# arbellea/LSTM-UNet

Measured on AMD Instinct MI355X. Metric: training frames/sec (seq_len*batch) at 256x256, higher is better.
Workload: dtype f32

## Files before the change

lstm-unet_amd/csrc/lu_conv.hip:

```cpp
#include <stdarg.h>
#include <stdlib.h>
#include <string.h>
#include <stdio.h>
#include <type_traits>
#include <utility>
#include "lu_device.h"

namespace {

constexpr int CK = 16;
constexpr int BM = 256;
constexpr int A_LD = CK + 4;

struct SrcInfo {
    const float* x;
    const float* w;
    int64_t frame_stride;
    int64_t w_tap_stride;
    int32_t pix_stride, C, w_row_stride;
    int32_t thin;
    int32_t nchunk;
    int32_t bf16;
};

// ... 234 lines not shown
            rok = row < CK && j < a.kk * si.C;
            tap = j / si.C;
            c = j - tap * si.C;
        }
        const float* wp = si.w + (int64_t)tap * si.w_tap_stride + (int64_t)c * si.w_row_stride + bcol;
        if (BVEC) {
            const bool ok = rok && ((EPI == LU_EPI_LSTM) || bcol < a.N);
            return *reinterpret_cast<const float4*>(ok ? wp : zp);
        } else {
            const float t0 = *((rok && bcol + 0 < a.N) ? wp + 0 : zp), t1 = *((rok && bcol + 1 < a.N) ? wp + 1 : zp),
                        t2 = *((rok && bcol + 2 < a.N) ? wp + 2 : zp), t3 = *((rok && bcol + 3 < a.N) ? wp + 3 : zp);
            return make_float4(t0, t1, t2, t3);
        }
    };
    auto load_weights = [&](const SrcInfo& si, bool thin, int tap_v, int chunk) {
        rb0 = load_w(si, thin, tap_v, chunk, 0);
        if (NPB > 1) rb1 = load_w(si, thin, tap_v, chunk, 1);
    };
    int64_t rowoff[RA];
#pragma unroll
    for (int i = 0; i < RA; ++i) rowoff[i] = 0;
    int cached_s = -1;
    auto load_stage = [&](const IterState& st) {
        const SrcInfo& si = a.src[st.s];
        const int c = st.chunk * CK + 4 * q;
        const bool cok = c < si.C;
        const float* pv[RA];
        if (GEN) {
#pragma unroll
            for (int i = 0; i < RA; ++i) {
                const int vy = vy0[i] + st.kh, vx = vx0[i] + st.kw;
                const int iy = vy >> a.dsh, ix = vx >> a.dsh;
                const bool ok = cok && vy >= 0 && vx >= 0 && iy < a.Hin && ix < a.Win && ((vy | vx) & a.dsh) == 0;
                const float* p = si.x + (int64_t)fr[i] * si.frame_stride + ((int64_t)iy * a.Win + ix) * si.pix_stride + c;
                pv[i] = ok ? p : zp;
            }
        } else {
            if (st.s != cached_s) {
                cached_s = st.s;
#pragma unroll
                for (int i = 0; i < RA; ++i)
                    rowoff[i] = (int64_t)fr[i] * si.frame_stride + ((int64_t)vy0[i] * a.Win + vx0[i]) * si.pix_stride;
            }
            const float* tapbase = si.x + ((int64_t)st.kh * a.Win + st.kw) * si.pix_stride + c;
#pragma unroll
            for (int i = 0; i < RA; ++i) {
                const bool ok = cok && (unsigned)(vy0[i] + st.kh) < (unsigned)a.Hin &&
                                (unsigned)(vx0[i] + st.kw) < (unsigned)a.Win;
                pv[i] = ok ? tapbase + rowoff[i] : zp;
            }
        }
#pragma unroll
        for (int i = 0; i < RA; ++i) ra[i] = *reinterpret_cast<const float4*>(pv[i]);
        load_weights(si, false, st.tap, st.chunk);
    };
    auto dma_stage = [&](const IterState& st, int buf) {
        const SrcInfo& si = a.src[st.s];
        if (!GEN && st.s != cached_s) {
            cached_s = st.s;
#pragma unroll
            for (int i = 0; i < RA; ++i)
                rowoff[i] = (int64_t)fr[i] * si.frame_stride + ((int64_t)vy0[i] * a.Win + vx0[i]) * si.pix_stride;
        }
        const float* tapbase = si.x + ((int64_t)st.kh * a.Win + st.kw) * si.pix_stride;
#pragma unroll
        for (int i = 0; i < RA; ++i) {
            const int row = (tid >> 2) + (NT / 4) * i;
            const int c = st.chunk * CK + 4 * (q ^ ((row >> 2) & 3));
            const float* p;
            bool ok;
            if (GEN) {
                const int vy = vy0[i] + st.kh, vx = vx0[i] + st.kw;
                const int iy = vy >> a.dsh, ix = vx >> a.dsh;
                ok = c < si.C && vy >= 0 && vx >= 0 && iy < a.Hin && ix < a.Win && ((vy | vx) & a.dsh) == 0;
                p = si.x + (int64_t)fr[i] * si.frame_stride + ((int64_t)iy * a.Win + ix) * si.pix_stride + c;
            } else {
                ok = c < si.C && (unsigned)(vy0[i] + st.kh) < (unsigned)a.Hin && (unsigned)(vx0[i] + st.kw) < (unsigned)a.Win;
                p = tapbase + rowoff[i] + c;
            }
            lu_glds16(ok ? p : zp, &As[buf][(wave * 16 + (NT / 4) * i) * ALD]);
        }
#pragma unroll
        for (int pp = 0; pp < NPB; ++pp) {
            const int row = brow0 + RPP * pp;
            const int c = st.chunk * CK + row;
            const bool ok = row < CK && c < si.C && ((EPI == LU_EPI_LSTM) || bcol < a.N);
            const float* wp = si.w + (int64_t)st.tap * si.w_tap_stride + (int64_t)c * si.w_row_stride + bcol;
            if (RPP * (pp + 1) <= CK || row < CK) lu_glds16(ok ? wp : zp, &Bs[buf][(wave * 64 + NT * pp) * 4]);
        }
    };

    auto load_thin = [&](const SrcInfo& si, int chunk) {
        const int kkC = a.kk * si.C;
        int dy[4], dx[4], cc[4];
        bool jok[4];
#pragma unroll
        for (int e = 0; e < 4; ++e) {
            int j = chunk * CK + 4 * q + e;
            jok[e] = j < kkC;
            int tap = j / si.C;
            cc[e] = j - tap * si.C;
            dy[e] = tap / a.k;
            dx[e] = tap - dy[e] * a.k;
        }
#pragma unroll
        for (int i = 0; i < RA; ++i) {
            float v[4];
#pragma unroll
            for (int e = 0; e < 4; ++e) {
                const int vy = vy0[i] + dy[e], vx = vx0[i] + dx[e];
                const int iy = vy >> a.dsh, ix = vx >> a.dsh;
                const bool ok = jok[e] && vy >= 0 && vx >= 0 && iy < a.Hin && ix < a.Win && ((vy | vx) & a.dsh) == 0;
                const float* p = si.x + (int64_t)fr[i] * si.frame_stride + ((int64_t)iy * a.Win + ix) * si.pix_stride + cc[e];
                v[e] = *(ok ? p : zp);
            }
            ra[i] = make_float4(v[0], v[1], v[2], v[3]);
        }
        load_weights(si, true, 0, chunk);
    };

    auto store_stage = [&](int buf) {
#pragma unroll
        for (int i = 0; i < RA; ++i)
        {
            const int row = (tid >> 2) + (NT / 4) * i;
            const int slot = DMA ? (q ^ ((row >> 2) & 3)) : q;
            *reinterpret_cast<float4*>(&As[buf][row * ALD + 4 * slot]) = ra[i];
        }
        if (RPP <= CK || brow0 < CK) *reinterpret_cast<float4*>(&Bs[buf][brow0 * BN + 4 * bq]) = rb0;
        if (NPB > 1) *reinterpret_cast<float4*>(&Bs[buf][(brow0 + RPP) * BN + 4 * bq]) = rb1;
    };

    f32x16 acc[MF][NF];
#pragma unroll
    for (int mf = 0; mf < MF; ++mf)
#pragma unroll
        for (int nf = 0; nf < NF; ++nf)
#pragma unroll
            for (int r = 0; r < 16; ++r) acc[mf][nf][r] = 0.f;

    const int arow = wave * (32 * MF) + (lane & 31);
    const int khalf = 4 * (lane >> 5);
    float4 afr[MF][2];
    float bvr[2][NF];
    auto rd_af = [&](int buf, int s) {
#pragma unroll
        for (int mf = 0; mf < MF; ++mf) {
            const int row = arow + 32 * mf;
            const int grp = 2 * s + (khalf >> 2);
            const int slot = DMA ? (grp ^ ((row >> 2) & 3)) : grp;
            afr[mf][s] = *reinterpret_cast<const float4*>(&As[buf][row * ALD + 4 * slot]);
        }
    };
    auto rd_bv = [&](int buf, int g) {
        const int s = g >> 2, j = g & 3;
#pragma unroll
        for (int nf = 0; nf < NF; ++nf) bvr[g & 1][nf] = Bs[buf][(8 * s + khalf + j) * BN + 32 * nf + (lane & 31)];
    };
    auto stage_begin = [&](int buf) {
        rd_af(buf, 0);
        rd_bv(buf, 0);
        rd_af(buf, 1);
    };
    auto mma_group = [&](int buf, int g) {
        const int s = g >> 2, j = g & 3;
        if (g + 1 < 8) rd_bv(buf, g + 1);
#pragma unroll
        for (int mf = 0; mf < MF; ++mf) {
            const float4& fa = afr[mf][s];
            const float av = j == 0 ? fa.x : j == 1 ? fa.y : j == 2 ? fa.z : fa.w;
#pragma unroll
            for (int nf = 0; nf < NF; ++nf) acc[mf][nf] = lu_mfma(av, bvr[g & 1][nf], acc[mf][nf]);
        }
    };
    auto mma_stage = [&](int buf) {
        stage_begin(buf);
#pragma unroll
        for (int g = 0; g < 8; ++g) mma_group(buf, g);
    };

    for (int ts = 0; ts < (ks == 0 ? a.n_thin : 0); ++ts) {
        const SrcInfo& si = a.tsrc[ts];
        for (int ch = 0; ch < si.nchunk; ++ch) {
            load_thin(si, ch);
            store_stage(0);
            __syncthreads();
            mma_stage(0);
            __syncthreads();
        }
    }

    int it0 = 0, it1 = a.n_it;
    if (a.ksplit > 1) {
        const int per = (a.n_it + a.ksplit - 1) / a.ksplit;
        it0 = ks * per;
        it1 = it0 + per < a.n_it ? it0 + per : a.n_it;
    }
    if (it1 > it0) {
        IterState st{0, 0, 0, 0, 0};
        {
            int r = it0;
            while (r >= a.src[st.s].nchunk * a.kk) {
                r -= a.src[st.s].nchunk * a.kk;
                ++st.s;
            }
            st.chunk = r / a.kk;
            st.tap = r - st.chunk * a.kk;
            st.kh = st.tap / a.k;
            st.kw = st.tap - st.kh * a.k;
        }
        if (DMA) {
            dma_stage(st, 0);
        } else {
            load_stage(st);
            store_stage(0);
        }
        __syncthreads();
        for (int it = it0; it < it1; ++it) {
            const int buf = (it - it0) & 1;
            stage_begin(buf);
            mma_group(buf, 0);
            LU_SCHED_FENCE();
            if (it + 1 < it1) iter_advance(st, a);
            if (DMA) {
                if (!LU_DBG(a, 1)) dma_stage(st, buf ^ 1);
                LU_SCHED_FENCE();
#pragma unroll
                for (int g = 1; g < 8; ++g) {
                    mma_group(buf, g);
                    LU_SCHED_FENCE();
                }
            } else {
                if (!LU_DBG(a, 1)) load_stage(st);
                LU_SCHED_FENCE();
#pragma unroll
                for (int g = 1; g < 7; ++g) {
                    mma_group(buf, g);
                    LU_SCHED_FENCE();
                }
                if (!LU_DBG(a, 2)) store_stage(buf ^ 1);
                LU_SCHED_FENCE();
                mma_group(buf, 7);
            }
            if (!LU_DBG(a, 4)) __syncthreads();
        }
    }

    if (EPI == LU_EPI_BIAS && a.out_vec4s && a.ksplit <= 1) {
        float* const Exw = &As[0][0] + wave * (16 * 36);
        const int cq = lane & 7;
#pragma unroll
        for (int mf = 0; mf < MF; ++mf)
#pragma unroll
            for (int half = 0; half < 2; ++half) {
                int64_t obase[2];
                bool rok[2];
#pragma unroll
                for (int q = 0; q < 2; ++q) {
                    const int64_t m = m0 + wave * (32 * MF) + mf * 32 + 16 * half + (lane >> 3) + 8 * q;
                    rok[q] = m < a.M;
                    RowCursor rc;
                    rc.set(a, rok[q] ? m : 0);
                    obase[q] = (int64_t)rc.f * a.out_frame_stride +
                               (a.out_row_stride ? (int64_t)rc.oy * a.out_row_stride + (int64_t)rc.ox * a.out_pix_stride
                                                 : (int64_t)rc.pix * a.out_pix_stride);
                }
#pragma unroll
                for (int nf = 0; nf < NF; ++nf) {
#pragma unroll
                    for (int rr = 0; rr < 8; ++rr)
                        Exw[((rr & 3) + 8 * (rr >> 2) + 4 * (lane >> 5)) * 36 + (lane & 31)] = acc[mf][nf][8 * half + rr];
                    LU_WAVE_SYNC();
                    const int col = n0 + 32 * nf + 4 * cq;
                    const float4 bq = (a.bias && col < a.N) ? *reinterpret_cast<const float4*>(a.bias + col) : make_float4(0.f, 0.f, 0.f, 0.f);
#pragma unroll
                    for (int q = 0; q < 2; ++q) {
                        float4 v = *reinterpret_cast<const float4*>(&Exw[((lane >> 3) + 8 * q) * 36 + 4 * cq]);
                        v.x += bq.x; v.y += bq.y; v.z += bq.z; v.w += bq.w;
                        if (rok[q] && col < a.N) *reinterpret_cast<float4*>(a.out + obase[q] + col) = v;
                    }
                    LU_WAVE_SYNC();
                }
            }
        return;
    }
#pragma unroll
    for (int mf = 0; mf < MF; ++mf) {
        const int64_t mb = m0 + wave * (32 * MF) + mf * 32 + 4 * (lane >> 5);
        RowCursor rc;
        rc.set(a, mb < a.M ? mb : 0);
#pragma unroll
        for (int r = 0; r < 16; ++r) {
            if (r) rc.advance(a, (r & 3) ? 1 : 5);
            const int64_t m = mb + (r & 3) + 8 * (r >> 2);
            if (m >= a.M) continue;
            float v[NF];
#pragma unroll
            for (int nf = 0; nf < NF; ++nf) v[nf] = acc[mf][nf][r];
            conv_epilogue_row<NF, EPI>(a, v, rc.f, rc.pix, m, nt, n0, ks, lane & 31, rc.oy);
        }
    }
}

template <int K, int EPI, bool ST = false>
__global__ __launch_bounds__(512, 4) void conv_halo_kernel(ConvArgs a) {
    const float* const lu_z16 = a.zero16 ? a.zero16 : lu_zero16;
    constexpr int NF = 4, BN = 128, NT = 512, TH = 8, TW = 32;
    constexpr int HWD = TW + K - 1, HHT = TH + K - 1, HP = HHT * HWD;
    constexpr int HPASS = (HP * 4 + NT - 1) / NT;
    constexpr int PAD = (K - 1) / 2;
    static_assert(HP * A_LD >= BM * A_LD, "halo buffer doubles as the [256][20] tile of the thin-source prologue");
    __shared__ __attribute__((aligned(16))) float Ah[HP * A_LD];
    __shared__ __attribute__((aligned(16))) float Bs[3][CK * BN];

    const int tid = threadIdx.x, lane = tid & 63, wave = tid >> 6;
    const int bid = blockIdx.x;
    const int slot = bid >> 3;
    int tile, nt, ks;
    const bool live = lu_block_tile(a, tile, nt, ks);
    if (a.xcd_by_n) {
        const int g = a.n_tiles >> 3;
        nt = (bid & 7) * g + (slot % g);
        tile = slot / g;
        if (tile >= a.m_tiles) return;
    } else if (!live) {
        return;
    }
    const int f = tile / a.tiles_pf;
    const int t2 = tile - f * a.tiles_pf;
    const int y0 = (t2 / a.tiles_x) * TH, x0 = (t2 % a.tiles_x) * TW;
    const int n0 = nt * BN;
    const float* const zp = lu_z16;
    const float* const x_s0 = a.src[0].x + (int64_t)f * a.src[0].frame_stride;
    const float* const x_s1 = a.src[1].x + (int64_t)f * a.src[1].frame_stride;
    const float* const w_s0 = a.src[0].w;
    const float* const w_s1 = a.src[1].w;
    const int64_t wts_s0 = a.src[0].w_tap_stride, wts_s1 = a.src[1].w_tap_stride;
    const int wrs_s0 = a.src[0].w_row_stride, wrs_s1 = a.src[1].w_row_stride;
    const int ps_s0 = a.src[0].pix_stride, ps_s1 = a.src[1].pix_stride;
    const int C_s0 = a.src[0].C, C_s1 = a.src[1].C;
    const int nch_s0 = a.src[0].nchunk, nch_s1 = a.src[1].nchunk;
    const int q = tid & 3;
    const int bq = tid & 31, brow = tid >> 5;
    const int bcol = (EPI == LU_EPI_LSTM) ? (bq >> 3) * a.F + nt * 32 + 4 * (bq & 7) : n0 + 4 * bq;

    lu_u4 rh[HPASS];
    float4 rb = make_float4(0.f, 0.f, 0.f, 0.f);
    auto load_halo = [&](int src, int chunk) {
        const int c = chunk * CK + 4 * q;
        const float* base = (src ? x_s1 : x_s0) + c;
        const int ps = src ? ps_s1 : ps_s0;
        const bool cok = c < (src ? C_s1 : C_s0);
#pragma unroll
        for (int i = 0; i < HPASS; ++i) {
            const int hp = (tid + NT * i) >> 2;
            const int hy = hp / HWD, hx = hp - hy * HWD;
            const int iy = y0 + hy - PAD, ix = x0 + hx - PAD;
            const bool ok = cok && hp < HP && iy >= 0 && iy < a.Hin && ix >= 0 && ix < a.Win;
            const float* p = base + (int64_t)(iy * a.Win + ix) * ps;
            rh[i] = *reinterpret_cast<const lu_u4*>(ok ? p : zp);
        }
    };
    auto store_halo = [&]() {
#pragma unroll
        for (int i = 0; i < HPASS; ++i) {
            const int hp = (tid + NT * i) >> 2;
            if (hp < HP) *reinterpret_cast<lu_u4*>(&Ah[hp * A_LD + 4 * q]) = rh[i];
        }
    };
    auto load_b = [&](const SrcInfo& si, bool thin, int tap_v, int chunk) {
        int tap, c;
        bool rok;
        if (!thin) {
            tap = tap_v;
            c = chunk * CK + brow;
            rok = c < si.C;
        } else {
            const int j = chunk * CK + brow;
            rok = j < a.kk * si.C;
            tap = j / si.C;
            c = j - tap * si.C;
        }
        const float* wp = si.w + (int64_t)tap * si.w_tap_stride + (int64_t)c * si.w_row_stride + bcol;
        const bool ok = rok && ((EPI == LU_EPI_LSTM) || bcol < a.N);
        rb = *reinterpret_cast<const float4*>(ok ? wp : zp);
    };
    int d_s = 0, d_chunk = 0, d_tap = 0;
    int64_t d_wts = 0;
    const float* wq = nullptr;
    bool wok = false;
    const bool colok = (EPI == LU_EPI_LSTM) || bcol < a.N;
    auto dma_seek = [&](int src, int chunk, int tap) {
        d_s = src;
        d_chunk = chunk;
        d_tap = tap;
        const int c = chunk * CK + brow;
        wq = (src ? w_s1 : w_s0) + (int64_t)tap * (src ? wts_s1 : wts_s0) + (int64_t)c * (src ? wrs_s1 : wrs_s0) + bcol;
        wok = c < (src ? C_s1 : C_s0) && colok;
        d_wts = src ? wts_s1 : wts_s0;
    };
    auto dma_next = [&](float* Bd) {
        lu_glds16(wok ? wq : zp, Bd + wave * 256);
        if (++d_tap < K * K) {
            wq += d_s ? wts_s1 : wts_s0;
        } else if (d_chunk + 1 < (d_s ? nch_s1 : nch_s0)) {
            dma_seek(d_s, d_chunk + 1, 0);
        } else {
            dma_seek(d_s + 1, 0, 0);
        }
    };
    auto dma_issue = [&](float* Bd, int mode) {
        if (mode == 0) {
            dma_next(Bd);
            return;
        }
        lu_glds16(wok ? wq : zp, Bd + wave * 256);
        if (mode == 1) wq += d_wts;
        else if (d_chunk + 1 < (d_s ? nch_s1 : nch_s0)) dma_seek(d_s, d_chunk + 1, 0);
        else dma_seek(d_s + 1, 0, 0);
    };
    auto store_b = [&](int buf) { *reinterpret_cast<float4*>(&Bs[buf][brow * BN + 4 * bq]) = rb; };

    f32x16 acc[NF];
#pragma unroll
    for (int nf = 0; nf < NF; ++nf)
#pragma unroll
        for (int r = 0; r < 16; ++r) acc[nf][r] = 0.f;

    const int khalf = 4 * (lane >> 5);
    const int boff = khalf * BN + (lane & 31);
    struct B4 {
        float x, y, z, w;
    };
    auto rd_b = [&](const float* Br, int g) {
        if (EPI == LU_EPI_BIAS) {
            const float4 v = *reinterpret_cast<const float4*>(Br + khalf * BN + 4 * (lane & 31) + (8 * (g >> 2) + (g & 3)) * BN);
            return B4{v.x, v.y, v.z, v.w};
        }
        const float* p = Br + boff + (8 * (g >> 2) + (g & 3)) * BN;
        return B4{p[0], p[32], p[64], p[96]};
    };
    auto rd_a = [&](int arow, int s) { return *reinterpret_cast<const float4*>(&Ah[arow * A_LD + 8 * s + khalf]); };
    auto mma4 = [&](float av, const B4& b) {
        acc[0] = lu_mfma(av, b.x, acc[0]);
        acc[1] = lu_mfma(av, b.y, acc[1]);
        acc[2] = lu_mfma(av, b.z, acc[2]);
        acc[3] = lu_mfma(av, b.w, acc[3]);
    };
    float4 fa0, fa1;
    B4 fb[2];
    auto fa_of = [&](int g) {
        const float4& fa = (g >> 2) ? fa1 : fa0;
        const int j = g & 3;
        return j == 0 ? fa.x : j == 1 ? fa.y : j == 2 ? fa.z : fa.w;
    };
    auto simple_stage = [&](const float* Br, int arow) {
        fa0 = rd_a(arow, 0);
        fa1 = rd_a(arow, 1);
#pragma unroll
        for (int g = 0; g < 8; ++g) {
            fb[0] = rd_b(Br, g);
            mma4(fa_of(g), fb[0]);
        }
    };

    if (ks == 0) {
        const int oyr[2] = {y0 + ((tid >> 2) >> 5), y0 + (((tid >> 2) + 128) >> 5)};
        const int oxr = x0 + ((tid >> 2) & 31);
        for (int ts = 0; ts < a.n_thin; ++ts) {
            const SrcInfo& si = a.tsrc[ts];
            const int kkC = a.kk * si.C;
            for (int ch = 0; ch < si.nchunk; ++ch) {
                float4 rt[2];
#pragma unroll
                for (int i = 0; i < 2; ++i) {
                    float v[4];
#pragma unroll
                    for (int e = 0; e < 4; ++e) {
                        const int jj = ch * CK + 4 * q + e;
                        const int tap = jj / si.C, cc = jj - tap * si.C;
                        const int dy = tap / K, dx = tap - dy * K;
                        const int iy = oyr[i] + dy - PAD, ix = oxr + dx - PAD;
                        const bool ok = jj < kkC && oyr[i] < a.Hin && oxr < a.Win && iy >= 0 && iy < a.Hin && ix >= 0 &&
                                        ix < a.Win;
                        const float* p = si.x + (int64_t)f * si.frame_stride + ((int64_t)iy * a.Win + ix) * si.pix_stride + cc;
                        v[e] = *(ok ? p : zp);
                    }
                    rt[i] = make_float4(v[0], v[1], v[2], v[3]);
                }
                load_b(si, true, 0, ch);
#pragma unroll
                for (int i = 0; i < 2; ++i)
                    *reinterpret_cast<float4*>(&Ah[((tid >> 2) + 128 * i) * A_LD + 4 * q]) = rt[i];
                store_b(0);
                __syncthreads();
                simple_stage(&Bs[0][0], wave * 32 + (lane & 31));
                __syncthreads();
            }
        }
    }

    int it0 = 0, it1 = a.n_it;
    if (a.ksplit > 1) {
        const int per = ST ? ((a.n_it / (K * K) + a.ksplit - 1) / a.ksplit) * (K * K) : (a.n_it + a.ksplit - 1) / a.ksplit;
        it0 = ks * per < a.n_it ? ks * per : a.n_it;
        it1 = it0 + per < a.n_it ? it0 + per : a.n_it;
    }
    if (it1 > it0) {
        IterState st{0, 0, 0, 0, 0};
        {
            int r = it0;
            while (r >= a.src[st.s].nchunk * a.kk) {
                r -= a.src[st.s].nchunk * a.kk;
                ++st.s;
            }
            st.chunk = r / a.kk;
            st.tap = r - st.chunk * a.kk;
            st.kh = st.tap / K;
            st.kw = st.tap - st.kh * K;
        }
        int c_s = st.s, c_chunk = st.chunk, tap = st.tap, kw = st.kw, aoff = st.kh * HWD + st.kw;
        auto next_chunk = [&](int& ns, int& nc) {
            ns = c_s;
            nc = c_chunk + 1;
            if (nc == (c_s ? nch_s1 : nch_s0)) {
                nc = 0;
                ++ns;
            }
        };
        load_halo(c_s, c_chunk);
        dma_seek(c_s, c_chunk, tap);
        dma_next(&Bs[0][0]);
        if (it0 + 1 < it1) dma_next(&Bs[1][0]);
        store_halo();
        if (it0 + 1 < it1 && tap == K * K - 1) {
            int ns, nc;
            next_chunk(ns, nc);
            load_halo(ns, nc);
        }
        __syncthreads();
        auto stage_sync = [&](int vm, bool lds) {
#ifdef LU_EMU
            __syncthreads();
#else
            if (lds) {
                if (vm == 0) __builtin_amdgcn_s_waitcnt(0x0070);
                else __builtin_amdgcn_s_waitcnt(0x0071);
            } else {
                if (vm == 0) __builtin_amdgcn_s_waitcnt(0x0F70);
                else __builtin_amdgcn_s_waitcnt(0x0F70 | HPASS);
            }
            __builtin_amdgcn_s_barrier();
#endif
        };
        auto stage = [&](float* __restrict__ Bd, const float* __restrict__ Br, const float* __restrict__ Bn, int arow, int arow_n,
                         bool dma, int dmode, bool halo_ld, bool halo_st, bool more) {
            fb[1] = rd_b(Br, 1);
            fa1 = rd_a(arow, 1);
            mma4(fa0.x, fb[0]);
            LU_SCHED_FENCE();
            if (halo_ld) {
                int ns, nc;
                next_chunk(ns, nc);
                load_halo(ns, nc);
            }
            LU_SCHED_FENCE();
#pragma unroll
            for (int g = 1; g < 4; ++g) {
                fb[(g + 1) & 1] = rd_b(Br, g + 1);
                mma4(fa_of(g), fb[g & 1]);
                LU_SCHED_FENCE();
            }
            if (!halo_st) {
                stage_sync(halo_ld ? 1 : 0, false);
                if (dma) dma_issue(Bd, dmode);
            }
            LU_SCHED_FENCE();
#pragma unroll
            for (int g = 4; g < 8; ++g) {
                if (g < 7) fb[(g + 1) & 1] = rd_b(Br, g + 1);
                else if (more && !halo_st) fb[0] = rd_b(Bn, 0);
                if (g == 5 && more && !halo_st) fa0 = rd_a(arow_n, 0);
                mma4(fa_of(g), fb[g & 1]);
                LU_SCHED_FENCE();
            }
            if (halo_st) {
#ifdef LU_EMU
                __syncthreads();
#else
                __builtin_amdgcn_s_barrier();
#endif
                store_halo();
                if (dma) dma_issue(Bd, dmode);
                stage_sync(dma ? 1 : 0, true);
                if (more) {
                    fa0 = rd_a(arow_n, 0);
                    fb[0] = rd_b(Bn, 0);
                }
            }
        };
        int b0 = 0, b1 = 1, b2 = 2;
        const int arow0 = wave * HWD + (lane & 31);
        fa0 = rd_a(arow0 + aoff, 0);
        fb[0] = rd_b(&Bs[0][0], 0);
        if constexpr (ST) {
            const int n_chunks = (it1 - it0) / (K * K);
            auto rotate = [&]() {
                const int t = b0;
                b0 = b1;
                b1 = b2;
                b2 = t;
            };
            for (int ci = 0; ci < n_chunks; ++ci) {
                const bool has_next = ci + 1 < n_chunks;
                int rowb = arow0;
                for (int kh = 0; kh < K - 1; ++kh) {
                    lu_static_for<K>([&](auto kc) {
                        constexpr int kw_ = decltype(kc)::value;
                        stage(&Bs[b2][0], &Bs[b0][0], &Bs[b1][0], rowb + kw_, kw_ + 1 < K ? rowb + kw_ + 1 : rowb + HWD, true, 1, false,
                              false, true);
                        rotate();
                    });
                    rowb += HWD;
                }
                lu_static_for<K>([&](auto kc) {
                    constexpr int kw_ = decltype(kc)::value;
                    stage(&Bs[b2][0], &Bs[b0][0], &Bs[b1][0], rowb + kw_, kw_ + 1 < K ? rowb + kw_ + 1 : arow0, has_next || kw_ + 2 < K,
                          kw_ == K - 3 ? 2 : 1, kw_ == K - 2 && has_next, kw_ == K - 1 && has_next, has_next || kw_ + 1 < K);
                    rotate();
                });
                next_chunk(c_s, c_chunk);
            }
        } else {
        for (int it = it0; it < it1; ++it) {
            const bool dma = it + 2 < it1, last_tap = tap == K * K - 1;
            int aoff_n = aoff + 1;
            if (kw + 1 == K) aoff_n += HWD - K;
            if (last_tap) aoff_n = 0;
            stage(&Bs[b2][0], &Bs[b0][0], &Bs[b1][0], arow0 + aoff, arow0 + aoff_n, dma, 0, dma && tap == K * K - 2,
                  it + 1 < it1 && last_tap, it + 1 < it1);
            aoff = aoff_n;
            if (++kw == K) kw = 0;
            if (++tap == K * K) {
                tap = 0;
                next_chunk(c_s, c_chunk);
            }
            const int t = b0;
            b0 = b1;
            b1 = b2;
            b2 = t;
        }
        }
        if (EPI == LU_EPI_LSTM) __syncthreads();
    }

    const int oy = y0 + wave;
    if (EPI == LU_EPI_BIAS) {
        const int col = n0 + 4 * (lane & 31);
        const bool slab = a.ksplit > 1;
        const bool vec = (a.N & 3) == 0 && (slab ? (reinterpret_cast<uintptr_t>(a.ws) & 15) == 0 : a.out_vec4 != 0);
        float4 b4 = make_float4(0.f, 0.f, 0.f, 0.f);
        if (!slab && a.bias) {
            if (col + 3 < a.N) {
                b4 = make_float4(a.bias[col], a.bias[col + 1], a.bias[col + 2], a.bias[col + 3]);
            } else {
                if (col < a.N) b4.x = a.bias[col];
                if (col + 1 < a.N) b4.y = a.bias[col + 1];
                if (col + 2 < a.N) b4.z = a.bias[col + 2];
            }
        }
#pragma unroll
        for (int r = 0; r < 16; ++r) {
            const int ox = x0 + (r & 3) + 8 * (r >> 2) + 4 * (lane >> 5);
            if (oy >= a.Hin || ox >= a.Win || col >= a.N) continue;
            const int64_t pix = (int64_t)oy * a.Win + ox;
            float* op;
            if (slab) {
                op = a.ws + ((int64_t)ks * a.M + (int64_t)f * a.HWo + pix) * a.N + col;
            } else if (a.out_row_stride) {
                op = a.out + (int64_t)f * a.out_frame_stride + (int64_t)oy * a.out_row_stride + (int64_t)ox * a.out_pix_stride + col;
            } else {
                op = a.out + (int64_t)f * a.out_frame_stride + pix * a.out_pix_stride + col;
            }
            const float4 v = make_float4(acc[0][r] + b4.x, acc[1][r] + b4.y, acc[2][r] + b4.z, acc[3][r] + b4.w);
            if (vec) {
                *reinterpret_cast<float4*>(op) = v;
            } else {
                op[0] = v.x;
                if (col + 1 < a.N) op[1] = v.y;
                if (col + 2 < a.N) op[2] = v.z;
                if (col + 3 < a.N) op[3] = v.w;
            }
        }
        return;
    }
    if (EPI == LU_EPI_LSTM && a.lstm_vec4 && NF == 4 && HP * A_LD >= 8 * (8 * 132)) {
        float* const Exw = Ah + wave * (8 * 132);
        const int F = a.F;
        const int lp = lane >> 3, cq = lane & 7;
        const int ch = nt * 32 + 4 * cq;
        const float* const bp = a.bias ? a.bias + ch : lu_z16;
        const int bst = a.bias ? F : 0;
#pragma unroll
        for (int qt = 0; qt < 4; ++qt) {
            const bool okp = oy < a.Hin && x0 + 8 * qt + lp < a.Win;
            const float4 cp = *reinterpret_cast<const float4*>(
                okp ? a.c_prev + (int64_t)f * a.c_prev_fs + ((int64_t)oy * a.Win + x0 + 8 * qt + lp) * F + ch : lu_z16);
            const float4 bi = *reinterpret_cast<const float4*>(bp), bf = *reinterpret_cast<const float4*>(bp + bst),
                         bg = *reinterpret_cast<const float4*>(bp + 2 * bst), bo = *reinterpret_cast<const float4*>(bp + 3 * bst);
#pragma unroll
            for (int nf = 0; nf < NF; ++nf)
#pragma unroll
                for (int rr = 0; rr < 4; ++rr)
                    Exw[(rr + 4 * (lane >> 5)) * 132 + 32 * nf + (lane & 31)] = acc[nf][4 * qt + rr];
            LU_WAVE_SYNC();
            const float* ex = &Exw[lp * 132 + 4 * cq];
            const int ox = x0 + 8 * qt + lp;
            const int64_t pix = (int64_t)oy * a.Win + ox;
            float* const gp = a.gates_out ? a.gates_out + (int64_t)f * a.gates_fs + pix * (4 * F) + ch : nullptr;
            float4 z, gi, gf, gg, go, cn, hn;
            z = *reinterpret_cast<const float4*>(ex);
            gi.x = hard_sigmoid(z.x + bi.x); gi.y = hard_sigmoid(z.y + bi.y); gi.z = hard_sigmoid(z.z + bi.z); gi.w = hard_sigmoid(z.w + bi.w);
            if (okp && gp) *reinterpret_cast<float4*>(gp) = gi;
            z = *reinterpret_cast<const float4*>(ex + 32);
            gf.x = hard_sigmoid(z.x + bf.x); gf.y = hard_sigmoid(z.y + bf.y); gf.z = hard_sigmoid(z.z + bf.z); gf.w = hard_sigmoid(z.w + bf.w);
            if (okp && gp) *reinterpret_cast<float4*>(gp + F) = gf;
            z = *reinterpret_cast<const float4*>(ex + 64);
            gg.x = lu_tanh_fast(z.x + bg.x); gg.y = lu_tanh_fast(z.y + bg.y); gg.z = lu_tanh_fast(z.z + bg.z); gg.w = lu_tanh_fast(z.w + bg.w);
            if (okp && gp) *reinterpret_cast<float4*>(gp + 2 * F) = gg;
            cn.x = fmaf(gf.x, cp.x, gi.x * gg.x); cn.y = fmaf(gf.y, cp.y, gi.y * gg.y);
            cn.z = fmaf(gf.z, cp.z, gi.z * gg.z); cn.w = fmaf(gf.w, cp.w, gi.w * gg.w);
            if (okp) *reinterpret_cast<float4*>(a.c_out + (int64_t)f * a.c_out_fs + pix * F + ch) = cn;
            z = *reinterpret_cast<const float4*>(ex + 96);
            go.x = hard_sigmoid(z.x + bo.x); go.y = hard_sigmoid(z.y + bo.y); go.z = hard_sigmoid(z.z + bo.z); go.w = hard_sigmoid(z.w + bo.w);
            if (okp && gp) *reinterpret_cast<float4*>(gp + 3 * F) = go;
            hn.x = go.x * lu_tanh_fast(cn.x); hn.y = go.y * lu_tanh_fast(cn.y); hn.z = go.z * lu_tanh_fast(cn.z); hn.w = go.w * lu_tanh_fast(cn.w);
            if (okp) *reinterpret_cast<float4*>(a.h_out + (int64_t)f * a.h_fs + pix * F + ch) = hn;
            LU_WAVE_SYNC();
        }
        return;
    }
#pragma unroll
    for (int r = 0; r < 16; ++r) {
        const int ox = x0 + (r & 3) + 8 * (r >> 2) + 4 * (lane >> 5);
        if (oy >= a.Hin || ox >= a.Win) continue;
        const int64_t pix = (int64_t)oy * a.Win + ox;
        float v[NF];
#pragma unroll
        for (int nf = 0; nf < NF; ++nf) v[nf] = acc[nf][r];
        conv_epilogue_row<NF, EPI>(a, v, f, pix, (int64_t)f * a.HWo + pix, nt, n0, ks, lane & 31);
    }
}

constexpr int CKB = 32;
constexpr int LDB = CKB + 8;

__device__ __forceinline__ void pack_weights_bf16_body(const float* __restrict__ w, int64_t tap_stride, int row_stride, int kk,
                                                       int C, int N, unsigned short* __restrict__ out, int64_t first, int64_t step) {
    const int nchunk = (C + CKB - 1) / CKB, nfr = (N + 31) / 32;
    const int64_t total = (int64_t)kk * nchunk * nfr * 128;
    for (int64_t i = first; i < total; i += step) {
        const int ln = (int)(i & 63), j = (int)((i >> 6) & 1);
        int64_t t = i >> 7;
        const int fr = (int)(t % nfr);
        t /= nfr;
        const int chunk = (int)(t % nchunk);
        const int tap = (int)(t / nchunk);
        const int n = fr * 32 + (ln & 31);
        const int c0 = chunk * CKB + 16 * j + 8 * (ln >> 5);
        const float* src = w + (int64_t)tap * tap_stride + (int64_t)c0 * row_stride + n;
        unsigned short v[8];
#pragma unroll
        for (int e = 0; e < 8; ++e)
            v[e] = (c0 + e < C && n < N) ? lu_f2bf(src[(int64_t)e * row_stride]) : (unsigned short)0;
        lu_u4 pk;
        pk.x = (unsigned)v[0] | ((unsigned)v[1] << 16);
        pk.y = (unsigned)v[2] | ((unsigned)v[3] << 16);
        pk.z = (unsigned)v[4] | ((unsigned)v[5] << 16);
        pk.w = (unsigned)v[6] | ((unsigned)v[7] << 16);
        *reinterpret_cast<lu_u4*>(out + (i << 3)) = pk;
    }
}

__global__ void pack_weights_bf16_kernel(const float* __restrict__ w, int64_t tap_stride, int row_stride, int kk, int C,
                                         int N, unsigned short* __restrict__ out) {
    pack_weights_bf16_body(w, tap_stride, row_stride, kk, C, N, out, (int64_t)blockIdx.x * blockDim.x + threadIdx.x,
                           (int64_t)gridDim.x * blockDim.x);
}

__global__ void pack_weights_split6_bf16_kernel(const float* __restrict__ w, int64_t tap_stride, int row_stride, int kk, int C, int cp,
                                                int N, unsigned order, unsigned short* __restrict__ out) {
    const int C6 = 6 * cp;
    const int nchunk = (C6 + CKB - 1) / CKB, nfr = (N + 31) / 32;
    const int64_t total = (int64_t)kk * nchunk * nfr * 128;
    for (int64_t i = (int64_t)blockIdx.x * blockDim.x + threadIdx.x; i < total; i += (int64_t)gridDim.x * blockDim.x) {
        const int ln = (int)(i & 63), j = (int)((i >> 6) & 1);
        int64_t t = i >> 7;
        const int fr = (int)(t % nfr);
        t /= nfr;
        const int chunk = (int)(t % nchunk);
        const int tap = (int)(t / nchunk);
        const int n = fr * 32 + (ln & 31);
        const int c0 = chunk * CKB + 16 * j + 8 * (ln >> 5);
        unsigned short v[8];
#pragma unroll
        for (int e = 0; e < 8; ++e) {
            const int ca = c0 + e, blk = ca / cp, c = ca - blk * cp;
            float hi = 0.f, mid = 0.f, lo = 0.f;
            if (ca < C6 && c < C && n < N) lu_split3(w[(int64_t)tap * tap_stride + (int64_t)c * row_stride + n], hi, mid, lo);
            const unsigned pc = (order >> (2 * (blk < 6 ? blk : 0))) & 3u;
            v[e] = lu_f2bf(pc == 0 ? hi : (pc == 1 ? mid : lo));
        }
        lu_u4 pk;
        pk.x = (unsigned)v[0] | ((unsigned)v[1] << 16);
        pk.y = (unsigned)v[2] | ((unsigned)v[3] << 16);
        pk.z = (unsigned)v[4] | ((unsigned)v[5] << 16);
        pk.w = (unsigned)v[6] | ((unsigned)v[7] << 16);
        *reinterpret_cast<lu_u4*>(out + (i << 3)) = pk;
    }
}

template <int EPI, int RW, int NFR = 4>
__device__ __forceinline__ void frag_epilogue(const ConvArgs& a, f32x16 (&acc)[RW], unsigned char* Ah, int f, int y0, int x0,
                                              int nt, int n0, int ks) {
    constexpr int BN = 32 * NFR, TW = 32, EX_LD = BN + 4;
    const int tid = threadIdx.x, lane = tid & 63, wave = tid >> 6;
    const int wm = wave / NFR, wn = wave % NFR;
    if (LU_DBG(a, 8)) {
        float t = 0.f;
#pragma unroll
        for (int i = 0; i < RW; ++i)
#pragma unroll
            for (int r = 0; r < 16; ++r) t += acc[i][r];
        if (t == 12345.678f) a.out[0] = t;
        return;
    }
    if (EPI == LU_EPI_LSTM) {
        float* Ex = reinterpret_cast<float*>(Ah);
        const int F = a.F;
        const int pr = tid >> 3, cq = tid & 7;
        const int g = pr >> 5, px = pr & 31;
        const int ch = nt * 32 + 4 * cq;
        float4 bi = make_float4(0.f, 0.f, 0.f, 0.f), bf = bi, bg = bi, bo = bi;
        if (a.bias) {
            bi = *reinterpret_cast<const float4*>(a.bias + ch);
            bf = *reinterpret_cast<const float4*>(a.bias + F + ch);
            bg = *reinterpret_cast<const float4*>(a.bias + 2 * F + ch);
            bo = *reinterpret_cast<const float4*>(a.bias + 3 * F + ch);
        }
        float4 cpv[RW];
#pragma unroll
        for (int i = 0; i < RW; ++i) {
            const int oy = y0 + RW * g + i, ox = x0 + px;
            const bool ok = oy < a.Hin && ox < a.Win;
            cpv[i] = *reinterpret_cast<const float4*>(ok ? a.c_prev + (int64_t)f * a.c_prev_fs + ((int64_t)oy * a.Win + ox) * F + ch
                                                         : (a.zero16 ? a.zero16 : lu_zero16));
        }
#pragma unroll
        for (int i = 0; i < RW; ++i) {
            __syncthreads();
#pragma unroll
            for (int r = 0; r < 16; ++r) {
                const int pxr = (r & 3) + 8 * (r >> 2) + 4 * (lane >> 5);
                Ex[(wm * TW + pxr) * EX_LD + 32 * wn + (lane & 31)] = acc[i][r];
            }
            __syncthreads();
            const int oy = y0 + RW * g + i, ox = x0 + px;
            if (oy >= a.Hin || ox >= a.Win) continue;
            const int64_t pix = (int64_t)oy * a.Win + ox;
            const float* ex = &Ex[(g * TW + px) * EX_LD + 4 * cq];
            const float4 zi = *reinterpret_cast<const float4*>(ex), zf = *reinterpret_cast<const float4*>(ex + 32),
                         zg = *reinterpret_cast<const float4*>(ex + 64), zo = *reinterpret_cast<const float4*>(ex + 96);
            const float4 cp = cpv[i];
            float4 gi, gf, gg, go, cn, hn;
#define LU_GATE(m)                                      \
    gi.m = hard_sigmoid(zi.m + bi.m);                   \
    gf.m = hard_sigmoid(zf.m + bf.m);                   \
    gg.m = lu_tanh_fast(zg.m + bg.m);                   \
    go.m = hard_sigmoid(zo.m + bo.m);                   \
    cn.m = fmaf(gf.m, cp.m, gi.m * gg.m);               \
    hn.m = go.m * lu_tanh_fast(cn.m);
            LU_GATE(x) LU_GATE(y) LU_GATE(z) LU_GATE(w)
#undef LU_GATE
            *reinterpret_cast<float4*>(a.c_out + (int64_t)f * a.c_out_fs + pix * F + ch) = cn;
            *reinterpret_cast<float4*>(a.h_out + (int64_t)f * a.h_fs + pix * F + ch) = hn;
            if (a.h16_out && a.h16_split) {
                float4 hh, hm, hl;
                lu_split3(hn.x, hh.x, hm.x, hl.x);
                lu_split3(hn.y, hh.y, hm.y, hl.y);
                lu_split3(hn.z, hh.z, hm.z, hl.z);
                lu_split3(hn.w, hh.w, hm.w, hl.w);
                lu_u2 vh, vm, vl;
                vh.x = lu_pack2bf(hh.x, hh.y); vh.y = lu_pack2bf(hh.z, hh.w);
                vm.x = lu_pack2bf(hm.x, hm.y); vm.y = lu_pack2bf(hm.z, hm.w);
                vl.x = lu_pack2bf(hl.x, hl.y); vl.y = lu_pack2bf(hl.z, hl.w);
                unsigned short* hp = a.h16_out + (int64_t)f * a.h16_fs + pix * (6 * F) + ch;
                *reinterpret_cast<lu_u2*>(hp) = vl;
                *reinterpret_cast<lu_u2*>(hp + F) = vm;
                *reinterpret_cast<lu_u2*>(hp + 2 * F) = vh;
                *reinterpret_cast<lu_u2*>(hp + 3 * F) = vm;
                *reinterpret_cast<lu_u2*>(hp + 4 * F) = vh;
                *reinterpret_cast<lu_u2*>(hp + 5 * F) = vh;
            } else if (a.h16_out) {
                lu_u2 hv;
                hv.x = lu_pack2bf(hn.x, hn.y);
                hv.y = lu_pack2bf(hn.z, hn.w);
                *reinterpret_cast<lu_u2*>(a.h16_out + (int64_t)f * a.h16_fs + pix * F + ch) = hv;
            }
            if (a.gates_out) {
                if (a.gates_bf16) {
                    unsigned short* gp = reinterpret_cast<unsigned short*>(a.gates_out) + (int64_t)f * a.gates_fs + pix * (4 * F) + ch;
                    lu_u2 v;
                    v.x = lu_pack2bf(gi.x, gi.y); v.y = lu_pack2bf(gi.z, gi.w);
                    *reinterpret_cast<lu_u2*>(gp) = v;
                    v.x = lu_pack2bf(gf.x, gf.y); v.y = lu_pack2bf(gf.z, gf.w);
                    *reinterpret_cast<lu_u2*>(gp + F) = v;
                    v.x = lu_pack2bf(gg.x, gg.y); v.y = lu_pack2bf(gg.z, gg.w);
                    *reinterpret_cast<lu_u2*>(gp + 2 * F) = v;
                    v.x = lu_pack2bf(go.x, go.y); v.y = lu_pack2bf(go.z, go.w);
                    *reinterpret_cast<lu_u2*>(gp + 3 * F) = v;
                } else {
                    float* gp = a.gates_out + (int64_t)f * a.gates_fs + pix * (4 * F) + ch;
                    *reinterpret_cast<float4*>(gp) = gi;
                    *reinterpret_cast<float4*>(gp + F) = gf;
                    *reinterpret_cast<float4*>(gp + 2 * F) = gg;
                    *reinterpret_cast<float4*>(gp + 3 * F) = go;
                }
            }
        }
        return;
    }
    if (EPI == LU_EPI_BIAS && a.out_vec4 && a.ksplit <= 1) {
        float* const Exw = reinterpret_cast<float*>(Ah) + wave * (16 * 36);
        const int cq = lane & 7;
        const int col = n0 + 32 * wn + 4 * cq;
        const float4 bq = (a.bias && col < a.N) ? *reinterpret_cast<const float4*>(a.bias + col) : make_float4(0.f, 0.f, 0.f, 0.f);
        __syncthreads();
#pragma unroll
        for (int i = 0; i < RW; ++i) {
            const int oy = y0 + RW * wm + i;
#pragma unroll
            for (int half = 0; half < 2; ++half) {
#pragma unroll
                for (int rr = 0; rr < 8; ++rr)
                    Exw[((rr & 3) + 8 * (rr >> 2) + 4 * (lane >> 5)) * 36 + (lane & 31)] = acc[i][8 * half + rr];
                LU_WAVE_SYNC();
#pragma unroll
                for (int q = 0; q < 2; ++q) {
                    const int lp = (lane >> 3) + 8 * q;
                    const int ox = x0 + 16 * half + lp;
                    float4 v = *reinterpret_cast<const float4*>(&Exw[lp * 36 + 4 * cq]);
                    v.x += bq.x; v.y += bq.y; v.z += bq.z; v.w += bq.w;
                    if (oy < a.Hin && ox < a.Win && col < a.N)
                        *reinterpret_cast<float4*>(a.out + (int64_t)f * a.out_frame_stride +
                                                   ((int64_t)oy * a.Win + ox) * a.out_pix_stride + col) = v;
                }
                LU_WAVE_SYNC();
            }
// ... 1454 lines not shown
```

lstm-unet_amd/csrc/lu_device.h:

```cpp
#pragma once
#include <stdint.h>
#include <string.h>
#include "../../include/lstm_unet_hip.h"

#ifdef LU_EMU
#include <string>
#include "emu_runtime.h"
namespace lu_launch_record {
inline bool on = false;
inline std::string text;
inline void add(const char* kernel) {
    if (!on) return;
    text += kernel;
    text += '\n';
}
}
#define LU_LAUNCH(kernel, grid, block, stream, ...) \
    (lu_launch_record::add(#kernel), lu_emu::launch((grid), (block), [=]() { kernel(__VA_ARGS__); }))
#define LU_LAUNCH_DYN(kernel, grid, block, lds_bytes, stream, ...) LU_LAUNCH(kernel, grid, block, stream, __VA_ARGS__)
#define LU_DYN_LDS(type, name) type* name = reinterpret_cast<type*>(lu_emu::g_dyn_lds)
static inline f32x16 lu_mfma(float a, float b, f32x16 c) { return lu_emu::mfma_32x32x2(a, b, c); }
static inline f32x16 lu_mfma_bf16(lu_bf16x8 a, lu_bf16x8 b, f32x16 c) { return lu_emu::mfma_32x32x16_bf16(a, b, c); }
static inline lu_bf16x4 lu_lds_tr16(const unsigned short* p) { return lu_emu::lds_read_tr16_b64(p); }
static inline float lu_shfl_xor(float v, int m) { return lu_emu::shfl_xor(v, m); }
static inline float lu_shfl_down(float v, int d) { return lu_emu::shfl_down(v, d); }
static inline void lu_glds16(const float* gptr, float* lds_wave_base) {
    const int lane = lu_emu::g_rt.cur->lin & 63;
    memcpy(reinterpret_cast<char*>(lds_wave_base) + lane * 16, gptr, 16);
}
#define LU_CHECK_LAUNCH() 0
#define LU_SCHED_FENCE() ((void)0)
#define LU_SCHED_GROUP(mask, n) ((void)0)
#define LU_WAVE_SYNC() lu_emu::wave_barrier()
#define LU_UNIFORM(x) (x)
#else
#include <hip/hip_runtime.h>
#include <atomic>
typedef float f32x16 __attribute__((ext_vector_type(16)));
#define LU_MAX_DEVICES 64
static inline int lu_current_device() {
    int d = 0;
    if (hipGetDevice(&d) != hipSuccess || d < 0 || d >= LU_MAX_DEVICES) return -1;
    return d;
}
#define LU_SYMBOL_ADDRESS(sym)                                                                                       \
    ([]() -> const void* {                                                                                           \
        static std::atomic<const void*> lu_addr_[LU_MAX_DEVICES];                                                    \
        const int lu_d_ = lu_current_device();                                                                       \
        if (lu_d_ < 0) return nullptr;                                                                               \
        const void* lu_p_ = lu_addr_[lu_d_].load(std::memory_order_acquire);                                         \
        if (!lu_p_) {                                                                                                \
            void* lu_q_ = nullptr;                                                                                   \
            if (hipGetSymbolAddress(&lu_q_, HIP_SYMBOL(sym)) == hipSuccess && lu_q_) {                               \
                lu_addr_[lu_d_].store(lu_q_, std::memory_order_release);                                             \
                lu_p_ = lu_q_;                                                                                       \
            }                                                                                                        \
        }                                                                                                            \
        return lu_p_;                                                                                                \
    }())
#define LU_LAUNCH(kernel, grid, block, stream, ...) \
    hipLaunchKernelGGL(kernel, (grid), (block), 0, (hipStream_t)(stream), __VA_ARGS__)
#define LU_LAUNCH_DYN(kernel, grid, block, lds_bytes, stream, ...)                                                  \
    do {                                                                                                            \
        static std::atomic<unsigned long long> lu_dyn_ready_{0ull};                          \
        const int lu_dev_ = lu_current_device();                                                                    \
        const unsigned long long lu_bit_ = lu_dev_ < 0 ? 0ull : (1ull << lu_dev_);                                  \
        if (!(lu_dyn_ready_.load(std::memory_order_acquire) & lu_bit_) || !lu_bit_) {                               \
            (void)hipFuncSetAttribute(reinterpret_cast<const void*>(&kernel),                                       \
                                      hipFuncAttributeMaxDynamicSharedMemorySize, 160 * 1024);                      \
            lu_dyn_ready_.fetch_or(lu_bit_, std::memory_order_release);                                             \
        }                                                                                                           \
        hipLaunchKernelGGL(kernel, (grid), (block), (lds_bytes), (hipStream_t)(stream), __VA_ARGS__);               \
    } while (0)
#define LU_DYN_LDS(type, name) extern __shared__ __attribute__((aligned(16))) type name[]
__device__ __forceinline__ f32x16 lu_mfma(float a, float b, f32x16 c) {
    return __builtin_amdgcn_mfma_f32_32x32x2f32(a, b, c, 0, 0, 0);
}
typedef short lu_bf16x8 __attribute__((ext_vector_type(8)));
__device__ __forceinline__ f32x16 lu_mfma_bf16(lu_bf16x8 a, lu_bf16x8 b, f32x16 c) {
    typedef __bf16 hw_bf16x8 __attribute__((ext_vector_type(8)));
    return __builtin_amdgcn_mfma_f32_32x32x16_bf16(__builtin_bit_cast(hw_bf16x8, a), __builtin_bit_cast(hw_bf16x8, b), c, 0,
                                                   0, 0);
}
typedef short lu_bf16x4 __attribute__((ext_vector_type(4)));
__device__ __forceinline__ lu_bf16x4 lu_lds_tr16(const unsigned short* p) {
    return __builtin_amdgcn_ds_read_tr16_b64_v4i16((__attribute__((address_space(3))) lu_bf16x4*)p);
}
__device__ __forceinline__ float lu_shfl_xor(float v, int m) { return __shfl_xor(v, m, 64); }
__device__ __forceinline__ float lu_shfl_down(float v, int d) { return __shfl_down(v, d, 64); }
__device__ __forceinline__ void lu_glds16(const float* gptr, float* lds_wave_base) {
    __builtin_amdgcn_global_load_lds((const __attribute__((address_space(1))) void*)gptr,
                                     (__attribute__((address_space(3))) void*)lds_wave_base, 16, 0, 0);
}
#define LU_CHECK_LAUNCH() lu_check_launch()
#define LU_SCHED_GROUP(mask, n) __builtin_amdgcn_sched_group_barrier((mask), (n), 0)
#define LU_SCHED_FENCE()                      \
    do {                                      \
        __builtin_amdgcn_sched_barrier(0);    \
        asm volatile("" ::: "memory");        \
        __builtin_amdgcn_sched_barrier(0);    \
    } while (0)
#define LU_WAVE_SYNC()                                          \
    do {                                                        \
        __builtin_amdgcn_fence(__ATOMIC_ACQ_REL, "wavefront");   \
        __builtin_amdgcn_wave_barrier();                        \
    } while (0)
int lu_check_launch();
#define LU_UNIFORM(x) __builtin_amdgcn_readfirstlane(x)
#endif

__device__ __attribute__((aligned(16))) static float lu_zero16[4] = {0.f, 0.f, 0.f, 0.f};

typedef unsigned lu_u4 __attribute__((ext_vector_type(4)));
typedef unsigned lu_u2 __attribute__((ext_vector_type(2)));
__device__ __host__ static inline float lu_bits2f(unsigned u) {
    float f;
    memcpy(&f, &u, 4);
    return f;
}
__device__ __host__ static inline unsigned lu_f2bits(float f) {
    unsigned u;
    memcpy(&u, &f, 4);
    return u;
}

void lu_set_error(const char* fmt, ...);

#define LU_REQUIRE(cond, ...)          \
    do {                               \
        if (!(cond)) {                 \
            lu_set_error(__VA_ARGS__); \
            return 1;                  \
        }                              \
    } while (0)

static inline int64_t lu_cdiv(int64_t a, int64_t b) { return (a + b - 1) / b; }

#ifdef LU_EMU
static inline unsigned lu_pack2bf(float lo, float hi);
#else
__device__ __forceinline__ unsigned lu_pack2bf(float lo, float hi) {
    typedef __bf16 hw_bf16x2 __attribute__((ext_vector_type(2)));
    hw_bf16x2 v;
    v.x = (__bf16)lo;
    v.y = (__bf16)hi;
    return __builtin_bit_cast(unsigned, v);
}
#endif

#ifdef LU_EMU
static inline float lu_tanh_fast(float x) {
    const float ax = fabsf(x);
    const float e = exp2f(ax * 2.8853900817779268f);
    const float t = copysignf(1.f - 2.f / (e + 1.f), x);
    const float x2 = x * x;
    const float s = fmaf(x * x2, fmaf(x2, 0.13333333f, -0.33333334f), x);
    return ax < 0.1f ? s : t;
}
#else
__device__ __forceinline__ float lu_tanh_fast(float x) {
    const float ax = fabsf(x);
    const float e = __builtin_amdgcn_exp2f(ax * 2.8853900817779268f);
    const float t = copysignf(fmaf(-2.f, __builtin_amdgcn_rcpf(e + 1.f), 1.f), x);
    const float x2 = x * x;
    const float s = fmaf(x * x2, fmaf(x2, 0.13333333f, -0.33333334f), x);
    return ax < 0.1f ? s : t;
}
#endif

__device__ __host__ static inline unsigned short lu_f2bf(float f) {
    unsigned u;
    memcpy(&u, &f, 4);
    u += 0x7FFFu + ((u >> 16) & 1u);
    return (unsigned short)(u >> 16);
}
#ifdef LU_EMU
static inline unsigned lu_pack2bf(float lo, float hi) { return (unsigned)lu_f2bf(lo) | ((unsigned)lu_f2bf(hi) << 16); }
#endif

__device__ __host__ static inline void lu_split3(float x, float& hi, float& mid, float& lo) {
#if defined(__clang__)
#pragma clang fp contract(off)
#endif
    unsigned u = (unsigned)lu_f2bf(x) << 16;
    if ((u & 0x7F800000u) == 0x7F800000u) {
        unsigned xb;
        memcpy(&xb, &x, 4);
        if ((xb & 0x7F800000u) != 0x7F800000u) {
            u = (xb & 0x80000000u) | 0x7F7F0000u;
        } else {
            u = xb & 0xFFFF0000u;
            if ((xb & 0x007FFFFFu) && !(u & 0x007F0000u)) u |= 0x00400000u;
            memcpy(&hi, &u, 4);
            mid = 0.f;
            lo = 0.f;
            return;
        }
    }
    memcpy(&hi, &u, 4);
    const float r1 = x - hi;
    u = (unsigned)lu_f2bf(r1) << 16;
    memcpy(&mid, &u, 4);
    u = (unsigned)lu_f2bf(r1 - mid) << 16;
    memcpy(&lo, &u, 4);
}
```

Baseline: 61.33.

## Precompute halo pixel offsets and reorder halo loads after MFMA groups in conv_halo_kernel

Hoists the halo pixel index and bounds computation out of the per-chunk load loop into a per-thread array. It moves the next-chunk halo global loads to after the MFMA groups and the stage sync, and issues the weight DMA through inline asm so the compiler stops tracking it for waitcnt. Opaque asm barriers are added to cut register pressure from rematerialised tid-derived values, and the vmcnt wait is simplified. The goals are lower VGPR and ALU overhead and better overlap of loads with compute, at the risk of incorrect hand-managed waitcnt ordering for the untracked loads.

Result: no change. 61.94, median of 6 (+1.0%).

```diff
diff --git a/lstm-unet_amd/csrc/lu_conv.hip b/lstm-unet_amd/csrc/lu_conv.hip
--- a/lstm-unet_amd/csrc/lu_conv.hip
+++ b/lstm-unet_amd/csrc/lu_conv.hip
@@ -560,6 +560,12 @@
     }
 }
 
+__device__ __forceinline__ int lu_tid_now() {
+    int t = threadIdx.x;
+    LU_OPAQUE(t);
+    return t;
+}
+
 template <int K, int EPI, bool ST = false>
 __global__ __launch_bounds__(512, 4) void conv_halo_kernel(ConvArgs a) {
     const float* const lu_z16 = a.zero16 ? a.zero16 : lu_zero16;
@@ -571,7 +577,7 @@
     __shared__ __attribute__((aligned(16))) float Ah[HP * A_LD];
     __shared__ __attribute__((aligned(16))) float Bs[3][CK * BN];
 
-    const int tid = threadIdx.x, lane = tid & 63, wave = tid >> 6;
+    const int tid = threadIdx.x, lane_l = tid & 63, wave = LU_UNIFORM(tid >> 6);
     const int bid = blockIdx.x;
     const int slot = bid >> 3;
     int tile, nt, ks;
@@ -600,30 +606,38 @@
     const int nch_s0 = a.src[0].nchunk, nch_s1 = a.src[1].nchunk;
     const int q = tid & 3;
     const int bq = tid & 31, brow = tid >> 5;
-    const int bcol = (EPI == LU_EPI_LSTM) ? (bq >> 3) * a.F + nt * 32 + 4 * (bq & 7) : n0 + 4 * bq;
+    const int gate_F = a.F, n_cols = a.N;
+    auto bcol_of = [&](int bq_) { return (EPI == LU_EPI_LSTM) ? (bq_ >> 3) * gate_F + nt * 32 + 4 * (bq_ & 7) : n0 + 4 * bq_; };
+    const int bcol = bcol_of(bq);
 
     lu_u4 rh[HPASS];
+    int hpix[HPASS];
+#pragma unroll
+    for (int i = 0; i < HPASS; ++i) {
+        const int hp = (tid + NT * i) >> 2;
+        const int hy = hp / HWD, hx = hp - hy * HWD;
+        const int iy = y0 + hy - PAD, ix = x0 + hx - PAD;
+        hpix[i] = (hp < HP && iy >= 0 && iy < a.Hin && ix >= 0 && ix < a.Win) ? iy * a.Win + ix : -1;
+    }
     float4 rb = make_float4(0.f, 0.f, 0.f, 0.f);
     auto load_halo = [&](int src, int chunk) {
-        const int c = chunk * CK + 4 * q;
+        const int c = chunk * CK + 4 * (lu_tid_now() & 3);
         const float* base = (src ? x_s1 : x_s0) + c;
-        const int ps = src ? ps_s1 : ps_s0;
+        int ps = LU_UNIFORM(src ? ps_s1 : ps_s0);
+        LU_OPAQUE_UNIFORM(ps);
         const bool cok = c < (src ? C_s1 : C_s0);
 #pragma unroll
         for (int i = 0; i < HPASS; ++i) {
-            const int hp = (tid + NT * i) >> 2;
-            const int hy = hp / HWD, hx = hp - hy * HWD;
-            const int iy = y0 + hy - PAD, ix = x0 + hx - PAD;
-            const bool ok = cok && hp < HP && iy >= 0 && iy < a.Hin && ix >= 0 && ix < a.Win;
-            const float* p = base + (int64_t)(iy * a.Win + ix) * ps;
-            rh[i] = *reinterpret_cast<const lu_u4*>(ok ? p : zp);
+            const float* p = base + (int64_t)hpix[i] * ps;
+            rh[i] = *reinterpret_cast<const lu_u4*>((cok && hpix[i] >= 0) ? p : zp);
         }
     };
     auto store_halo = [&]() {
+        const int t = lu_tid_now();
+        float* const hst = &Ah[(t >> 2) * A_LD + 4 * (t & 3)];
 #pragma unroll
         for (int i = 0; i < HPASS; ++i) {
-            const int hp = (tid + NT * i) >> 2;
-            if (hp < HP) *reinterpret_cast<lu_u4*>(&Ah[hp * A_LD + 4 * q]) = rh[i];
+            if ((NT * (i + 1) - 1) / 4 < HP || ((t + NT * i) >> 2) < HP) *reinterpret_cast<lu_u4*>(hst + i * (NT / 4) * A_LD) = rh[i];
         }
     };
     auto load_b = [&](const SrcInfo& si, bool thin, int tap_v, int chunk) {
@@ -647,18 +661,18 @@
     int64_t d_wts = 0;
     const float* wq = nullptr;
     bool wok = false;
-    const bool colok = (EPI == LU_EPI_LSTM) || bcol < a.N;
     auto dma_seek = [&](int src, int chunk, int tap) {
         d_s = src;
         d_chunk = chunk;
         d_tap = tap;
-        const int c = chunk * CK + brow;
-        wq = (src ? w_s1 : w_s0) + (int64_t)tap * (src ? wts_s1 : wts_s0) + (int64_t)c * (src ? wrs_s1 : wrs_s0) + bcol;
-        wok = c < (src ? C_s1 : C_s0) && colok;
+        const int t = lu_tid_now();
+        const int c = chunk * CK + (t >> 5), col = bcol_of(t & 31);
+        wq = (src ? w_s1 : w_s0) + (int64_t)tap * (src ? wts_s1 : wts_s0) + (int64_t)c * (src ? wrs_s1 : wrs_s0) + col;
+        wok = c < (src ? C_s1 : C_s0) && ((EPI == LU_EPI_LSTM) || col < n_cols);
         d_wts = src ? wts_s1 : wts_s0;
     };
     auto dma_next = [&](float* Bd) {
-        lu_glds16(wok ? wq : zp, Bd + wave * 256);
+        lu_glds16_uncounted(wok ? wq : zp, Bd + wave * 256);
         if (++d_tap < K * K) {
             wq += d_s ? wts_s1 : wts_s0;
         } else if (d_chunk + 1 < (d_s ? nch_s1 : nch_s0)) {
@@ -672,7 +686,7 @@
             dma_next(Bd);
             return;
         }
-        lu_glds16(wok ? wq : zp, Bd + wave * 256);
+        lu_glds16_uncounted(wok ? wq : zp, Bd + wave * 256);
         if (mode == 1) wq += d_wts;
         else if (d_chunk + 1 < (d_s ? nch_s1 : nch_s0)) dma_seek(d_s, d_chunk + 1, 0);
         else dma_seek(d_s + 1, 0, 0);
@@ -685,14 +699,14 @@
 #pragma unroll
         for (int r = 0; r < 16; ++r) acc[nf][r] = 0.f;
 
-    const int khalf = 4 * (lane >> 5);
-    const int boff = khalf * BN + (lane & 31);
+    const int khalf = 4 * (lane_l >> 5);
+    const int boff = khalf * BN + (lane_l & 31);
     struct B4 {
         float x, y, z, w;
     };
     auto rd_b = [&](const float* Br, int g) {
         if (EPI == LU_EPI_BIAS) {
-            const float4 v = *reinterpret_cast<const float4*>(Br + khalf * BN + 4 * (lane & 31) + (8 * (g >> 2) + (g & 3)) * BN);
+            const float4 v = *reinterpret_cast<const float4*>(Br + khalf * BN + 4 * (lane_l & 31) + (8 * (g >> 2) + (g & 3)) * BN);
             return B4{v.x, v.y, v.z, v.w};
         }
         const float* p = Br + boff + (8 * (g >> 2) + (g & 3)) * BN;
@@ -752,7 +766,7 @@
                     *reinterpret_cast<float4*>(&Ah[((tid >> 2) + 128 * i) * A_LD + 4 * q]) = rt[i];
                 store_b(0);
                 __syncthreads();
-                simple_stage(&Bs[0][0], wave * 32 + (lane & 31));
+                simple_stage(&Bs[0][0], wave * 32 + (lane_l & 31));
                 __syncthreads();
             }
         }
@@ -791,6 +805,7 @@
         dma_next(&Bs[0][0]);
         if (it0 + 1 < it1) dma_next(&Bs[1][0]);
         store_halo();
+        LU_WAIT_VMEM_ALL();
         if (it0 + 1 < it1 && tap == K * K - 1) {
             int ns, nc;
             next_chunk(ns, nc);
@@ -806,7 +821,7 @@
                 else __builtin_amdgcn_s_waitcnt(0x0071);
             } else {
                 if (vm == 0) __builtin_amdgcn_s_waitcnt(0x0F70);
-                else __builtin_amdgcn_s_waitcnt(0x0F70 | HPASS);
+                else __builtin_amdgcn_s_waitcnt(0x0F71);
             }
             __builtin_amdgcn_s_barrier();
 #endif
@@ -817,21 +832,20 @@
             fa1 = rd_a(arow, 1);
             mma4(fa0.x, fb[0]);
             LU_SCHED_FENCE();
+#pragma unroll
+            for (int g = 1; g < 4; ++g) {
+                fb[(g + 1) & 1] = rd_b(Br, g + 1);
+                mma4(fa_of(g), fb[g & 1]);
+                LU_SCHED_FENCE();
+            }
+            if (!halo_st) {
+                stage_sync(0, false);
+                if (dma) dma_issue(Bd, dmode);
+            }
             if (halo_ld) {
                 int ns, nc;
                 next_chunk(ns, nc);
                 load_halo(ns, nc);
-            }
-            LU_SCHED_FENCE();
-#pragma unroll
-            for (int g = 1; g < 4; ++g) {
-                fb[(g + 1) & 1] = rd_b(Br, g + 1);
-                mma4(fa_of(g), fb[g & 1]);
-                LU_SCHED_FENCE();
-            }
-            if (!halo_st) {
-                stage_sync(halo_ld ? 1 : 0, false);
-                if (dma) dma_issue(Bd, dmode);
             }
             LU_SCHED_FENCE();
 #pragma unroll
@@ -858,7 +872,7 @@
             }
         };
         int b0 = 0, b1 = 1, b2 = 2;
-        const int arow0 = wave * HWD + (lane & 31);
+        const int arow0 = wave * HWD + (lane_l & 31);
         fa0 = rd_a(arow0 + aoff, 0);
         fb[0] = rd_b(&Bs[0][0], 0);
         if constexpr (ST) {
@@ -912,6 +926,7 @@
         if (EPI == LU_EPI_LSTM) __syncthreads();
     }
 
+    const int lane = lu_tid_now() & 63;
     const int oy = y0 + wave;
     if (EPI == LU_EPI_BIAS) {
         const int col = n0 + 4 * (lane & 31);
diff --git a/lstm-unet_amd/csrc/lu_device.h b/lstm-unet_amd/csrc/lu_device.h
--- a/lstm-unet_amd/csrc/lu_device.h
+++ b/lstm-unet_amd/csrc/lu_device.h
@@ -28,11 +28,15 @@
     const int lane = lu_emu::g_rt.cur->lin & 63;
     memcpy(reinterpret_cast<char*>(lds_wave_base) + lane * 16, gptr, 16);
 }
+static inline void lu_glds16_uncounted(const float* gptr, float* lds_wave_base) { lu_glds16(gptr, lds_wave_base); }
+#define LU_WAIT_VMEM_ALL() ((void)0)
 #define LU_CHECK_LAUNCH() 0
 #define LU_SCHED_FENCE() ((void)0)
 #define LU_SCHED_GROUP(mask, n) ((void)0)
 #define LU_WAVE_SYNC() lu_emu::wave_barrier()
 #define LU_UNIFORM(x) (x)
+#define LU_OPAQUE(x) ((void)0)
+#define LU_OPAQUE_UNIFORM(x) ((void)0)
 #else
 #include <hip/hip_runtime.h>
 #include <atomic>
@@ -92,6 +96,11 @@
     __builtin_amdgcn_global_load_lds((const __attribute__((address_space(1))) void*)gptr,
                                      (__attribute__((address_space(3))) void*)lds_wave_base, 16, 0, 0);
 }
+__device__ __forceinline__ void lu_glds16_uncounted(const float* gptr, float* lds_wave_base) {
+    const unsigned l = __builtin_amdgcn_readfirstlane((unsigned)(uintptr_t)(__attribute__((address_space(3))) void*)lds_wave_base);
+    asm volatile("s_mov_b32 m0, %1\n\ts_nop 0\n\tglobal_load_lds_dwordx4 %0, off" : : "v"(gptr), "s"(l) : "memory");
+}
+#define LU_WAIT_VMEM_ALL() __builtin_amdgcn_s_waitcnt(0x0F70)
 #define LU_CHECK_LAUNCH() lu_check_launch()
 #define LU_SCHED_GROUP(mask, n) __builtin_amdgcn_sched_group_barrier((mask), (n), 0)
 #define LU_SCHED_FENCE()                      \
@@ -107,6 +116,8 @@
     } while (0)
 int lu_check_launch();
 #define LU_UNIFORM(x) __builtin_amdgcn_readfirstlane(x)
+#define LU_OPAQUE(x) asm volatile("" : "+v"(x))
+#define LU_OPAQUE_UNIFORM(x) asm volatile("" : "+s"(x))
 #endif
 
 __device__ __attribute__((aligned(16))) static float lu_zero16[4] = {0.f, 0.f, 0.f, 0.f};
```
